# SNUCP/MKTFHE

Measured on AMD Instinct MI355X. Metric: NAND gate-bootstraps/sec, higher is better.
Workload: dtype f64

## Files before the change

mktfhe_amd/csrc/context.cpp:

```cpp
#include <hip/hip_runtime.h>

#include <algorithm>
#include <cstdio>
#include <cstdlib>
#include <cstring>
#include <string.h>
#include <cmath>
#include <memory>
#include <string>
#include <vector>

#include "device_api.h"
#include "device_mem.h"
#include "fft_device.h"
#include "host_internal.h"
#include "rng_chacha.h"
#include "../../include/mktfhe_ring_share.h"

using mktd::cplx;
using mkt::DevBuf;

namespace {
thread_local std::string g_create_error;

struct TimedSpan { int cls; hipEvent_t a, b; };

int env_int(const char *name, int dflt) { const char *v = getenv(name); return v ? atoi(v) : dflt; }
// ... 19 lines not shown
struct DevGuard {
    int prev = -1; bool ok = true;
    explicit DevGuard(int dev) { if (hipGetDevice(&prev) != hipSuccess) prev = -1; if (prev != dev) ok = hipSetDevice(dev) == hipSuccess; }
    ~DevGuard() { if (prev >= 0) (void)hipSetDevice(prev); }
};
Tune tune_from_env() { Tune t; for (const Switch &w : SWITCHES) t.*w.member = w.env ? env_int(w.env, w.dflt) : w.dflt; return t; }
}

thread_local const char *mktd::last_rot_kernel = "";
thread_local int mktd::last_rot_static_l = 0, mktd::last_rot_static_logB = 0;

const mktd::LaunchTuning &mktd::launch_tuning() {
    static const LaunchTuning t = [] {
        LaunchTuning q{};
        q.fft_grid = env_int("MKT_FFT_GRID", 0); q.fft_nb = env_int("MKT_FFT_NB", 1); q.fft_igrid = env_int("MKT_FFT_IGRID", 0);
        q.ks_g = env_int("MKT_KS_G", 32); q.ks_blocks = env_int("MKT_KS_BLOCKS", 0); q.ks_waves = env_int("MKT_KS_WAVES", 0); q.ks_pair = env_int("MKT_KS_PAIR", -1); q.ntt_grid = env_int("MKT_NTT_GRID", 0);
        return q;
    }();
    return t;
}

enum KeyTable { T_TW, T_MONOMIAL, T_BRK, T_KSK, T_PUB, T_CRS, T_RLK_D, T_RLK_F, T_SLOT_PARTY, T_SLOT_ROW, T_FX_TAB, T_FX_BRK, T_FX_STAT, T_NTT, T_COUNT };
struct ResidentTable {
    void **slot = nullptr; size_t elems = 0, esize = 0;
    bool per_party = false, present = false, cloned = false;
    size_t bytes(int nparty) const { return (per_party ? (size_t)nparty : 1) * elems * esize; }
};
struct KeySet {
    int device = 0;
    mkt::Twiddles tw;
    cplx *d_tw = nullptr;
    cplx *d_monomial = nullptr;
    cplx *d_brk = nullptr;
    uint32_t *d_ksk = nullptr; mkt::KskLayout ksk;
    cplx *d_rlk_d = nullptr, *d_rlk_f = nullptr, *d_pub = nullptr, *d_crs = nullptr;
    mkt::LoadedKeys loaded;
    int rtot = 1;
    int *d_slot_party = nullptr, *d_slot_row = nullptr;
    uint64_t *d_ntt = nullptr;
    cplx *d_fx_tab = nullptr;
    cplx *d_fx_brk = nullptr;
    unsigned long long *d_fx_stat = nullptr;
    double fx_kmax = 0.0;
    DevBuf d_pack; int pack_l = 0, pack_logB = 0; size_t pack_party_bytes = 0;
    std::vector<uint8_t> pack_loaded;
    ResidentTable tab[T_COUNT];
    DevBuf own[T_COUNT];
    size_t stride(KeyTable t) const { return tab[t].elems; }
    template <class T> T *party(KeyTable t, int party) const { return static_cast<T *>(*tab[t].slot) + (size_t)party * tab[t].elems; }
// ... 20 lines not shown
    int device = 0;
    int logM = 0, logN = 0, M = 0;
    int dev_order = MKT_DEVORDER;
    hipStream_t stream = nullptr;
    hipStream_t own_stream = nullptr;
    hipEvent_t moved = nullptr;
    std::string err;
    std::shared_ptr<KeySet> ks;
    bool exact = false;
    int split = 1;
    Workspace ws;
    bool timing = false;
    std::vector<TimedSpan> spans;
    Tune tune{};
    const char *last_rot_kernel = "";
    int rot_static_l = 0, rot_static_logB = 0;
    double pm_amax = 0.0;
    double pm_bound = -1.0;
    double fx_last_resid = 0.0;

    const cplx *fx_om() const { return ks->d_fx_tab; }
    const cplx *fx_tw() const { return ks->d_fx_tab + M; }
    const cplx *fx_nat() const { return ks->d_fx_tab + 2 * (size_t)M; }
    mktd::TwPtrs twp() const { return mktd::TwPtrs{ks->d_tw, ks->d_tw + M, ks->d_tw + 2 * (size_t)M, ks->d_tw + 3 * (size_t)M}; }
    bool keys_shared() const { return ks.use_count() > 1; }
};

namespace {

int fail(mkt_ctx *c, int code, const std::string &msg) { if (c) c->err = msg; else g_create_error = msg; return code; }
// ... 248 lines not shown
    mktd::RotArgs a = rot_args(c, lwe, stride, pre);
    a.init_mode = 0; a.out_mode = 0; a.acc_io = acc; a.ngates = B;
    if (route == Route::F64_KANY) HIPCHK(c, mktd::launch_blindrotate_kany(c->logM, p.W, p.k, a, scratch, B, c->stream));
    else if (route == Route::F64_KR) HIPCHK(c, mktd::launch_blindrotate_kr(c->logM, p.W, p.k, a, B, c->stream));
    else HIPCHK(c, mktd::launch_blindrotate_k1(c->logM, p.W, a, B, c->stream));
    return MKT_OK;
}

int do_keyswitch(mkt_ctx *c, const void *acc, uint32_t *out, size_t B, const uint32_t *src = nullptr, const uint32_t *coef = nullptr, size_t nacc = 0) {
    const mkt_params &p = c->p;
    mktd::KsArgs a{};
    a.src = src; a.coef = coef; a.nacc = nacc;
    a.acc = acc; a.out = out; a.ksk = c->ks->d_ksk; a.ksk_party_stride = c->ks->stride(T_KSK); a.n1p = c->ks->ksk.n1p;
    a.N = p.N; a.n = p.n; a.f = p.f; a.logD = p.logD; a.drows = c->sh.ksk_drows; a.kacc = c->sh.kacc;
    a.mk = mkt::is_mk(p.scheme) ? 1 : 0; a.balanced = mkt::is_block(p.scheme) ? 1 : 0; a.lmss = p.scheme == MKT_LMSS ? 1 : 0;
    size_t dw = 0, pw = 0;
    mktd::ks_scratch_words(a, B, &dw, &pw);
    HIPCHK(c, c->ws.ksd.reserve((dw + pw) * 4));
    if (dw) { a.digits = c->ws.ksd.as<uint32_t>(); a.partial = a.digits + dw; }
    Timer tm(c, 2);
    HIPCHK(c, mktd::launch_keyswitch(p.W, a, B, c->stream));
    return MKT_OK;
}

int rotate_chunk(mkt_ctx *c, const uint32_t *lin, size_t B) {
    const mkt_params &p = c->p;
    if (!mkt::is_kms(p.scheme)) {
        HIPCHK(c, mktd::launch_testvector(p.W, lin, c->sh.lwe_len, c->logN, c->sh.kacc, c->ws.acc.p, B, c->stream));
        return do_blindrotate(c, lin, c->sh.lwe_len, 0, nullptr, c->ws.acc.p, B);
    }
// ... 211 lines not shown
    auto row = [&](KeyTable t, auto &member, size_t elems, bool per_party, bool present, bool cloned) { ks.tab[t] = ResidentTable{(void **)&member, elems, sizeof(*member), per_party, present, cloned}; };
    row(T_TW,         ks.d_tw,         4 * M,                                                         false,     true,    true);
    row(T_MONOMIAL,   ks.d_monomial,   2 * N * M,                                                     false,     true,    true);
    row(T_BRK,        ks.d_brk,        (size_t)p.n * c->sh.brk_polys * tp,                            true,      true,    true);
    row(T_KSK,        ks.d_ksk,        ks.ksk.resident_words(),                                        true,      true,    true);
    row(T_PUB,        ks.d_pub,        (size_t)p.l_uni * tp,                                          true,      mk,      true);
    row(T_CRS,        ks.d_crs,        (size_t)p.l_uni * tp,                                          false,     mk,      true);
    row(T_RLK_D,      ks.d_rlk_d,      (size_t)p.l_uni * tp,                                          true,      kms,     true);
    row(T_RLK_F,      ks.d_rlk_f,      (size_t)p.l_uni * 2 * tp,                                      true,      kms,     true);
    row(T_SLOT_PARTY, ks.d_slot_party, (size_t)ks.rtot,                                               false,     true,    false);
    row(T_SLOT_ROW,   ks.d_slot_row,   (size_t)ks.rtot,                                               false,     true,    false);
    row(T_FX_TAB,     ks.d_fx_tab,     3 * M,                                                         false,     fx,      false);
    row(T_FX_BRK,     ks.d_fx_brk,     fx_per,                                                        true,      fx,      true);
    row(T_FX_STAT,    ks.d_fx_stat,    1,                                                             false,     fx,      true);
    row(T_NTT,        ks.d_ntt,        (N + 4) * 2,                                                   false,     c->exact, false);
}

constexpr int NO_PARTY = -1; enum class Gate { EXACT, F64_OR_EXACT_KMS };
int key_write_guard(mkt_ctx *c, bool ptrs_ok, int party, Gate gate, bool (*scheme_ok)(int) = nullptr) {
    if (!c || !ptrs_ok || (party != NO_PARTY && (party < 0 || party >= c->sh.nparty)) || (scheme_ok && !scheme_ok(c->p.scheme))) return fail(c, MKT_ERR_ARG, "bad argument");
    if (gate == Gate::EXACT) MKT_EXACT_GATE(c); else MKT_F64_OR_EXACT_KMS(c);
    return keys_writable(c);
}
hipError_t install_brk(mkt_ctx *c, int party, const void *src) {
    KeySet &ks = *c->ks;
    hipError_t e = to_resident(c, src, mkt::brk_polys_total(c->p, c->sh), ks.party<cplx>(T_BRK, party), false, ks.d_fx_brk ? ks.party<cplx>(T_FX_BRK, party) : nullptr);
    if (e == hipSuccess) e = hipStreamSynchronize(c->stream);
    if (e == hipSuccess && ks.d_fx_brk) e = fx_after_key_load(c);
    if (e == hipSuccess) ks.loaded.mark(mkt::K_BRK, party);
    return e;
}
hipError_t ksk_zero(mkt_ctx *c, int party) { return hipMemsetAsync(c->ks->party<uint32_t>(T_KSK, party), 0, c->ks->stride(T_KSK) * sizeof(uint32_t), c->stream); }
hipError_t ksk_repitch(mkt_ctx *c, uint32_t *dst, int dpitch, const uint32_t *src, int spitch, hipMemcpyKind kind) { return hipMemcpy2DAsync(dst, (size_t)dpitch * 4, src, (size_t)spitch * 4, (size_t)c->ks->ksk.n1 * 4, c->ks->ksk.rows, kind, c->stream); }
hipError_t ksk_to_resident(mkt_ctx *c, int party, const uint32_t *rows, hipMemcpyKind kind) { return ksk_repitch(c, c->ks->party<uint32_t>(T_KSK, party), c->ks->ksk.n1p, rows, c->ks->ksk.n1, kind); }
hipError_t ksk_to_rows(mkt_ctx *c, const uint32_t *padded, uint32_t *rows, hipMemcpyKind kind) { return ksk_repitch(c, rows, c->ks->ksk.n1, padded, c->ks->ksk.n1p, kind); }

}

extern "C" {

int mkt_abi_version(void) { return MKT_ABI_VERSION; }

const char *mkt_last_error(const mkt_ctx *ctx) { return ctx ? ctx->err.c_str() : g_create_error.c_str(); }

int mkt_ctx_create(const mkt_params *params, int arith_mode, int device, mkt_ctx **out) {
    if (!params || !out) return fail(nullptr, MKT_ERR_ARG, "null argument");
    *out = nullptr;
    std::string why;
    if (mkt::validate_params(*params, why)) return fail(nullptr, MKT_ERR_ARG, why);
    if (arith_mode != MKT_ARITH_F64REF && arith_mode != MKT_ARITH_EXACT) return fail(nullptr, MKT_ERR_ARG, "unknown arithmetic mode");
// ... 25 lines not shown
    DevGuard dg(device);
    auto bail = [&](int code) { std::string m = c->err; mkt_ctx_destroy(c); g_create_error = m; return code; };
    if (!dg.ok) { c->err = "hipSetDevice failed"; return bail(MKT_ERR_HIP); }
    const mkt_params &p = c->p;
    const int np = c->sh.nparty, M = c->M;
    c->ks->loaded.reset(np);
    mkt::make_twiddles(p.N, c->ks->tw);
    std::vector<int> sp, sr;
    if (mkt::is_kms(p.scheme)) {
        for (int i = 0; i < p.k; i++) { int rows = i == 0 ? 1 : p.l_lev; for (int r = 0; r < rows; r++) { sp.push_back(i); sr.push_back(r); } }
    } else { sp.push_back(0); sr.push_back(0); }
    c->ks->rtot = (int)sp.size();
    describe_key_set(c);
    if (c->ks->stride(T_BRK) * sizeof(cplx) > 0x7fffffffull) { c->err = "per-party bootstrapping key exceeds the 2 GiB window of the rotation kernels' buffer descriptors"; return bail(MKT_ERR_UNSUPPORTED); }
#define CK(call) do { hipError_t _e = (call); if (_e != hipSuccess) { c->err = std::string(#call) + ": " + hipGetErrorString(_e); return bail(_e == hipErrorOutOfMemory ? MKT_ERR_NOMEM : MKT_ERR_HIP); } } while (0)
    for (int t = 0; t < T_COUNT; t++) if (c->ks->tab[t].present) { CK(c->ks->own[t].alloc(c->ks->tab[t].bytes(np))); *c->ks->tab[t].slot = c->ks->own[t].p; }
    CK(hipMemcpy(c->ks->d_slot_party, sp.data(), sp.size() * sizeof(int), hipMemcpyHostToDevice));
    CK(hipMemcpy(c->ks->d_slot_row, sr.data(), sr.size() * sizeof(int), hipMemcpyHostToDevice));
    if (c->ks->d_fx_tab) {
        CK(hipMemset(c->ks->d_fx_stat, 0, 8));
        const size_t tb = (size_t)M * sizeof(cplx);
        CK(hipMemcpy(c->ks->d_fx_tab, c->ks->tw.fx_om.data(), tb, hipMemcpyHostToDevice));
        CK(hipMemcpy(c->ks->d_fx_tab + M, c->ks->tw.fx_tw.data(), tb, hipMemcpyHostToDevice));
        CK(hipMemcpy(c->ks->d_fx_tab + 2 * (size_t)M, c->ks->tw.fx_nat.data(), tb, hipMemcpyHostToDevice));
    }
#undef CK
    int r = upload_twiddles(c);
    if (!r && c->exact) r = upload_ntt_tables(c);
    if (!r) r = build_monomial(c);
    if (r) return bail(r);
    *out = c;
// ... 44 lines not shown
    if (!src || !dst) return MKT_ERR_ARG;
    if (std::memcmp(&src->p, &dst->p, sizeof(mkt_params)) != 0 || src->exact != dst->exact) return fail(dst, MKT_ERR_ARG, "key replication between contexts of different parameters");
    if (int w = keys_writable(dst)) return w;
    { DevGuard g(src->device); HIPCHK(dst, hipStreamSynchronize(src->stream)); }
    const int sd = src->device, dd = dst->device;
    KeySet &a = *src->ks, &b = *dst->ks;
    b.tw = a.tw;
    for (int t = 0; t < T_COUNT; t++)
        if (a.tab[t].cloned && a.tab[t].present && b.tab[t].present)
            HIPCHK(dst, (hipError_t)mkt_internal_copy_across(*b.tab[t].slot, dd, *a.tab[t].slot, sd, a.tab[t].bytes(src->sh.nparty), no_peer));
    if (a.d_fx_brk && b.d_fx_brk) b.fx_kmax = a.fx_kmax;
    b.loaded = a.loaded;
    dst->tune = src->tune;
    { DevGuard g(sd); HIPCHK(dst, hipDeviceSynchronize()); }
    { DevGuard g(dd); HIPCHK(dst, hipDeviceSynchronize()); }
    return MKT_OK;
}
#ifndef MKT_BUILD_ID
#define MKT_BUILD_ID "unknown"
#endif
const char *mkt_build_id(void) { return MKT_BUILD_ID; }
int mkt_internal_device_of(const mkt_ctx *c) { return c ? c->device : -1; }
size_t mkt_internal_lwe_len(const mkt_ctx *c) { return c ? (size_t)c->sh.lwe_len : 0; }
size_t mkt_internal_acc_bytes(const mkt_ctx *c) { return c ? (size_t)(1 + c->sh.kacc) * poly_bytes(c) : 0; }

int mkt_set_stream(mkt_ctx *c, void *hip_stream) {
    if (!c) return MKT_ERR_ARG;
    const hipStream_t next = (hipStream_t)hip_stream;
    if (next == c->stream) return MKT_OK;
    DevGuard dg(c->device);
    if (!c->moved) HIPCHK(c, hipEventCreateWithFlags(&c->moved, hipEventDisableTiming));
    HIPCHK(c, hipEventRecord(c->moved, c->stream));
// ... 15 lines not shown
            return fail(c, MKT_ERR_ARG, "mkt_set_option: " + k + " = " + std::to_string(value) + " is not one of " + list);
        }
        if (w.resets_workspace && c->tune.*w.member != value) c->ws.gates = 0;
        c->tune.*w.member = value;
        return MKT_OK;
    }
    return fail(c, MKT_ERR_ARG, "mkt_set_option: unknown option '" + k + "'");
}

const char *mkt_last_kernel_name(const mkt_ctx *c) { return c ? c->last_rot_kernel : ""; }

int mkt_get_metric(mkt_ctx *c, const char *name, double *out) {
    if (!c || !name || !out) return fail(c, MKT_ERR_ARG, "null argument");
    const std::string k(name);
    if (k == "fx_available") *out = fx_usable(c) ? 1.0 : 0.0;
    else if (k == "fx_bound") *out = c->ks->d_fx_brk ? fx_bound(c, c->ks->fx_kmax) : -1.0;
    else if (k == "fx_kmax") *out = c->ks->fx_kmax;
    else if (k == "fx_last_resid") *out = c->fx_last_resid;
    else if (k == "polymul_amax") *out = c->pm_amax;
    else if (k == "fx_polymul_bound") *out = c->pm_bound;
    else if (k == "rot_static_l") *out = c->rot_static_l;
    else if (k == "rot_static_logB") *out = c->rot_static_logB;
    else if (k == "mem_guard_check") {
        DevGuard dg(c->device);
        *out = (double)mkt::memguard::sweep(c->device);
        mkt::memguard::Finding f;
        if (mkt::memguard::last_finding(f)) c->err = mkt::memguard::text(f);
    }
    else if (k == "mem_guard_buffers") *out = (double)mkt::memguard::swept();
    else if (k == "mem_guard_released") *out = (double)mkt::memguard::released();
// ... 51 lines not shown
}

int mkt_load_brk(mkt_ctx *c, int party, const void *data, int fmt) {
    if (int r = key_write_guard(c, data != nullptr, party, Gate::EXACT)) return r;
    DevGuard dg(c->device);
    int r = upload_polys(c, data, mkt::brk_polys_total(c->p, c->sh), c->ks->party<cplx>(T_BRK, party), fmt, false, party);
    if (!r && fmt != MKT_FMT_INT_COEFF) c->ks->loaded.mark(mkt::K_BRK, party);
    return r;
}

int mkt_load_ksk(mkt_ctx *c, int party, const uint32_t *data) {
    if (int r = key_write_guard(c, data != nullptr, party, Gate::EXACT)) return r;
    DevGuard dg(c->device);
    HIPCHK(c, ksk_zero(c, party));
    HIPCHK(c, ksk_to_resident(c, party, data, hipMemcpyHostToDevice));
    HIPCHK(c, hipStreamSynchronize(c->stream));
    c->ks->loaded.mark(mkt::K_KSK, party);
    return MKT_OK;
}

int mkt_load_rlk(mkt_ctx *c, int party, const void *d, const void *f, int fmt) {
    if (int r = key_write_guard(c, d && f, party, Gate::F64_OR_EXACT_KMS, mkt::is_kms)) return r;
    DevGuard dg(c->device);
    const size_t l = (size_t)c->p.l_uni;
    int r = upload_polys(c, d, l, c->ks->party<cplx>(T_RLK_D, party), fmt);
    if (!r) r = upload_polys(c, f, 2 * l, c->ks->party<cplx>(T_RLK_F, party), fmt);
    if (!r) c->ks->loaded.mark(mkt::K_RLK, party);
    return r;
}

// ... 22 lines not shown
    DevGuard dg(c->device);
    const size_t brk_bytes = mkt::brk_polys_total(p, c->sh) * poly_bytes(c);
    DevBuf out, crs_int;
    DeviceSecret lwe{c}, z{c};
    mktd::KeygenArgs a{};
    hipError_t e = keygen_setup(c, K, crs, lwe, z, {{&out, brk_bytes}}, crs_int, a);
    if (e != hipSuccess) return hipfail(c, e, "device keygen setup");
    a.out = out.p; a.zoff = 0;
    if (!ring_keys_cover(c, K)) e = hipErrorInvalidValue;
    if (e == hipSuccess) e = mktd::launch_keygen_brk(a, unienc ? 1 : 0, c->stream);
    if (e == hipSuccess && brk_out) e = hipMemcpyAsync(brk_out, out.p, brk_bytes, hipMemcpyDeviceToHost, c->stream);
    if (e == hipSuccess) e = install_brk(c, party, out.p);
    if (e == hipSuccess) e = ksk_zero(c, party);
    a.zoff = mkt::is_kms(p.scheme) ? 1 : 0;
    if (e == hipSuccess) e = mktd::launch_keygen_ksk(a, c->ks->party<uint32_t>(T_KSK, party), c->ks->ksk.n1p, c->sh.ksk_kr, c->sh.ksk_drows, mkt::is_block(p.scheme) ? 1 : 0, c->stream);
    e = wipe_secrets(wipe_secrets(e, z, a), lwe, a);
    if (e != hipSuccess) return hipfail(c, e, "device keygen");
    c->ks->loaded.mark(mkt::K_KSK, party);
    if (ksk_out) return mkt_get_ksk(c, party, ksk_out);
    return MKT_OK;
}

int mkt_keygen_device(mkt_ctx *c, int party, const mkt_client_party *K, const void *crs) {
    return keygen_device_impl(c, party, K, crs, nullptr, nullptr);
}

int mkt_keygen_device_export(mkt_ctx *c, int party, const mkt_client_party *K, const void *crs, void *brk_out, uint32_t *ksk_out) {
    if (!brk_out || !ksk_out) return fail(c, MKT_ERR_ARG, "null output");
    return keygen_device_impl(c, party, K, crs, brk_out, ksk_out);
}
// ... 86 lines not shown
        a.log_units = c->logN + (p.W == 64 ? 1 : 0) - 4; a.body = sb.dev; a.out = dst; a.npolys = brk_polys_total;
        e = mktd::launch_seeded_brk_expand(a, c->stream);
        if (e == hipSuccess && load) e = install_brk(c, party, dst);
        if (e != hipSuccess) return hipfail(c, e, "seeded bootstrapping key expansion");
    }
    if (ksk_seeded) {
        if ((r = sk.in(ksk_seeded, rows * 4, mem, true))) return r;
        uint32_t *dst = c->ks->party<uint32_t>(T_KSK, party);
        if (!load) { HIPCHK(c, padded.alloc(c->ks->ksk.resident_words() * 4)); dst = padded.as<uint32_t>(); }
        mktd::SeededKskArgs a{};
        mkt::seed_to_key(mask_seed, a.mkey);
        a.party = party; a.n = p.n; a.n1p = c->ks->ksk.n1p; a.rows_per_cj = (uint32_t)(c->sh.ksk_drows * p.f);
        a.absent_below = mkt::is_block(p.scheme) ? p.n : 0; a.body = sk.as<const uint32_t>(); a.out = dst; a.rows = rows;
        e = mktd::launch_seeded_ksk_expand(a, c->stream);
        if (e == hipSuccess && !load) e = ksk_to_rows(c, dst, ksk_out, mem == MKT_MEM_HOST ? hipMemcpyDeviceToHost : hipMemcpyDeviceToDevice);
        if (e != hipSuccess) return hipfail(c, e, "seeded key-switching key expansion");
    }
    HIPCHK(c, hipStreamSynchronize(c->stream));
    if (!load) return brk_out ? so.out(brk_out) : MKT_OK;
    if (ksk_seeded) c->ks->loaded.mark(mkt::K_KSK, party);
    return MKT_OK;
}

int mkt_seeded_keys_expand(mkt_ctx *c, int party, const uint8_t *mask_seed, const void *brk_seeded, const uint32_t *ksk_seeded, void *brk_out, uint32_t *ksk_out, int mem) {
    return seeded_keys_impl(c, party, mask_seed, brk_seeded, ksk_seeded, false, brk_out, ksk_out, mem);
}

int mkt_load_seeded_keys(mkt_ctx *c, int party, const uint8_t *mask_seed, const void *brk_seeded, const uint32_t *ksk_seeded) {
    if (int r = key_write_guard(c, brk_seeded || ksk_seeded, NO_PARTY, Gate::EXACT)) return r;
    return seeded_keys_impl(c, party, mask_seed, brk_seeded, ksk_seeded, true, nullptr, nullptr, MKT_MEM_HOST);
// ... 791 lines not shown
```

mktfhe_amd/csrc/device_api.h:

```cpp
#pragma once
#include <hip/hip_runtime.h>
#include <stddef.h>
#include <stdint.h>

#include "rot_plan.h"

namespace mktd {

struct cplx;

struct TwPtrs { const cplx *psi, *psiinv, *roots, *rootsinv; };

struct LaunchTuning { int fft_grid, fft_nb, fft_igrid, ks_g, ks_blocks, ks_waves, ks_pair, ntt_grid; };
const LaunchTuning &launch_tuning();
extern thread_local const char *last_rot_kernel;
extern thread_local int last_rot_static_l, last_rot_static_logB;
inline void note_rot_kernel(const char *name, int static_l = 0, int static_logB = 0) {
    last_rot_kernel = name; last_rot_static_l = static_l; last_rot_static_logB = static_logB;
}

struct RotArgs {
    TwPtrs tw;
    const cplx *brk;
    size_t brk_party_stride;
    const cplx *monomial;
    const uint32_t *lwe;
    int lwe_stride;
    int pre_switched;
// ... 43 lines not shown
    const uint32_t *lwe;
    int lwe_stride, pre_switched;
    int n, logN, k, l, logB;
    const cplx *brk;
    size_t brk_party_stride;
    const cplx *pub_b;
    const cplx *crs;
    const cplx *monomial;
    void *acc;
    cplx *scratch;
    void *vscratch;
    int stagger;
    int dev_order;
};

struct KsArgs {
    const void *acc;
    uint32_t *out;
    const uint32_t *ksk;
    size_t ksk_party_stride;
    int n1p;
    int N, n, f, logD, drows;
    int kacc;
    int mk;
    int balanced;
    int lmss;
    uint32_t *digits;
    uint32_t *partial;
    const uint32_t *src;
    const uint32_t *coef;
    size_t nacc;
};
void ks_scratch_words(const KsArgs &a, size_t B, size_t *digit_words, size_t *partial_words);

struct KeygenArgs {
    uint32_t key[8];
    int party;
    int N, n, W;
    int kr, l, logB;
    int zoff;
    int f, logD;
    double sigma_ring, sigma_lwe;
    const uint32_t *lwekey;
    const int8_t *zring;
    const void *crs;
    void *out;
};
hipError_t launch_keygen_brk(const KeygenArgs &a, int unienc, hipStream_t s);
// ... 228 lines not shown
```

mktfhe_amd/csrc/host_internal.h:

```cpp
#pragma once
#include <cstddef>
#include <cstdint>
#include <cstring>
#include <string>
#include <vector>

#include "../../include/mktfhe.h"
#include "../../include/mktfhe_pack.h"

namespace mkt {

struct Twiddles {
    std::vector<double> psi, psiinv, roots, rootsinv;
    std::vector<double> fx_om, fx_tw, fx_nat;
};
void make_twiddles(int N, Twiddles &tw);

inline bool is_mk(int s) { return s == MKT_CCS || s == MKT_KMS || s == MKT_KMS_BLOCK; }
inline bool is_kms(int s) { return s == MKT_KMS || s == MKT_KMS_BLOCK; }
inline bool is_block(int s) { return s == MKT_LMSS || s == MKT_KMS_BLOCK; }

struct Shape {
    int nparty;
    int kr;
// ... 24 lines not shown
inline bool lut_nout_ok(int nout, int N) { return (nout == 1 || nout == 2 || nout == 4 || nout == 8) && nout <= N; }
inline bool lut_nu_ok(int nu, int N) { return nu >= 0 && nu <= 3 && (1 << nu) <= N; }
inline bool lut_ncoef_ok(size_t ncoef, int N) { return ncoef >= 1 && ncoef <= (size_t)N; }
inline bool host_below(const uint32_t *v, size_t n, size_t bound) {
    for (size_t j = 0; j < n; j++) if (v[j] >= bound) return false;
    return true;
}
inline size_t brk_seeded_polys(const mkt_params &p, const Shape &s) { return (size_t)p.n * (p.scheme == MKT_CCS ? 2 * (size_t)p.l_uni : (size_t)(s.kr + 1) * p.l_gsw); }
inline size_t ksk_rows(const mkt_params &p, const Shape &s) { return (size_t)s.ksk_kr * p.N * s.ksk_drows * p.f; }
inline size_t brk_polys_total(const mkt_params &p, const Shape &s) { return (size_t)p.n * s.brk_polys; }
struct KskLayout {
    size_t rows = 0; int n1 = 0, n1p = 0;
    size_t resident_words() const { return rows * (size_t)n1p; }
};
inline KskLayout ksk_layout(const mkt_params &p, const Shape &s) { return KskLayout{ksk_rows(p, s), p.n + 1, (p.n + 1 + 3) / 4 * 4}; }

enum KeyPiece { K_BRK, K_KSK, K_RLK, K_PUB, K_CRS };
struct LoadedKeys {
    std::vector<uint8_t> of;
    static constexpr unsigned bit(KeyPiece k) { return 1u << k; }
    void reset(int nparty) { of.assign((size_t)nparty, 0); }
    void mark(KeyPiece k, int party) { for (size_t i = 0; i < of.size(); i++) if (party < 0 || (size_t)party == i) of[i] |= (uint8_t)bit(k); }
    bool has_all(unsigned pieces, int party) const { return (of[(size_t)party] & pieces) == pieces; }
    bool has(KeyPiece k, int party) const { return has_all(bit(k), party < 0 ? 0 : party); }
    bool any_transformed() const {
        for (uint8_t m : of) if (m & (bit(K_BRK) | bit(K_RLK) | bit(K_PUB) | bit(K_CRS))) return true;
        return false;
    }
};
inline bool pack_gadget_ok(int l, int logB) { return logB >= 1 && logB <= 16 && l >= 1 && l * logB <= 32; }
// ... 40 lines not shown
```

mktfhe_amd/csrc/kernels.hip:

```cpp
#include "kernel_common.h"

#include <type_traits>

#pragma clang fp contract(off)

#ifdef MKT_TU
#define MKT_IN_TU(n) (MKT_TU == (n))
#else
#define MKT_IN_TU(n) 1
#endif

namespace mktd {

#if MKT_IN_TU(0)
constexpr int FFT_PF = 2;
typedef double __attribute__((ext_vector_type(2))) mkt_d2;
template <typename T> __device__ __forceinline__ T stream_load(const T *p) { return __builtin_nontemporal_load(p); }
__device__ __forceinline__ cplx stream_load_c(const cplx *p) {
    mkt_d2 v = __builtin_nontemporal_load(reinterpret_cast<const mkt_d2 *>(p));
    return cplx{v.x, v.y};
}
__device__ __forceinline__ void stream_store_c(cplx *p, cplx z) {
    mkt_d2 v = {z.re, z.im};
    __builtin_nontemporal_store(v, reinterpret_cast<mkt_d2 *>(p));
// ... 1567 lines not shown
        if (W == 64) return launch_ccs_one<LM, uint64_t, 0, 0>(a, B, s);
        if constexpr (LM == 9 || LM == 10) {
            if (a.l == 3 && a.logB == 8) return launch_ccs_one<LM, uint32_t, 3, 8>(a, B, s);
            if (a.l == 4 && a.logB == 8) return launch_ccs_one<LM, uint32_t, 4, 8>(a, B, s);
            if (a.l == 5 && a.logB == 6) return launch_ccs_one<LM, uint32_t, 5, 6>(a, B, s);
        }
        return launch_ccs_one<LM, uint32_t, 0, 0>(a, B, s);
    });
    return hipGetLastError();
}

#endif

#if MKT_IN_TU(0)
namespace {
struct KsPlan { int G, waves, ngroups, parties, gblocks, slabs, jslab; bool pair; };
KsPlan ks_plan(const KsArgs &a, size_t B, bool have_scratch) {
    KsPlan q{};
    q.G = 32;
    int target_blocks = 1024;
    if (a.balanced) target_blocks = a.mk ? 4096 : 8192;
    const LaunchTuning &lt = launch_tuning();
    if (lt.ks_g == 8 || lt.ks_g == 16) q.G = lt.ks_g;
    if (lt.ks_blocks > 0) target_blocks = lt.ks_blocks;
    q.pair = lt.ks_pair != 0 && a.logD == 2 && a.f % 2 == 0 && q.G == 32 && have_scratch;
    if (q.pair && lt.ks_blocks <= 0) target_blocks = 1024;
    q.ngroups = (int)((B + q.G - 1) / q.G);
    q.parties = a.mk ? a.kacc : 1;
    auto nslabs = [&] {
        int sl = (target_blocks + q.ngroups * q.parties - 1) / (q.ngroups * q.parties);
        if (sl < 1) sl = 1;
        if (sl > a.N / 8) sl = a.N / 8;
        return sl < 1 ? 1 : sl;
    };
    q.slabs = nslabs();
    q.jslab = (a.N + q.slabs - 1) / q.slabs;
    q.slabs = (a.N + q.jslab - 1) / q.jslab;
    q.waves = lt.ks_waves > 0 ? lt.ks_waves : 4;
    if (q.waves != 2 && q.waves != 4) q.waves = 1;
    if (q.G != 32) q.waves = 1;
    if (a.balanced && lt.ks_waves <= 0 && !q.pair) q.waves = 1;
    q.gblocks = (q.ngroups + q.waves - 1) / q.waves;
    return q;
}
}

void ks_scratch_words(const KsArgs &a, size_t B, size_t *digit_words, size_t *partial_words) {
    const KsPlan q = ks_plan(a, B, true);
    *digit_words = q.pair ? (size_t)a.kacc * q.ngroups * (size_t)a.N * 32 : 0;
    *partial_words = q.pair ? (size_t)q.slabs * q.parties * B * (size_t)a.n1p : 0;
}

template <bool AT>
static hipError_t launch_keyswitch_as(int W, const KsArgs &a, size_t B, hipStream_t s) {
    const KsPlan q = ks_plan(a, B, a.digits && a.partial);
    const int ngroups = q.ngroups;
    const dim3 grid((unsigned)(q.gblocks * q.slabs), (unsigned)q.parties, (unsigned)((a.n1p + KS_CHUNK_WORDS - 1) / KS_CHUNK_WORDS));
    const size_t ks_lds = q.pair ? (size_t)KS_STAGES * 16 * KS_LANES * sizeof(uint4) : (size_t)KS_STAGES * (1 + a.drows * (a.balanced ? 2 : 1)) * KS_LANES * sizeof(uint4);
    if (ks_lds > 64 * 1024) return hipErrorInvalidValue;
    const dim3 words(blocks_for(B * (size_t)ks_lwe_len(a), 256));
    using C1 = std::integral_constant<int, 1>; using C2 = std::integral_constant<int, 2>; using C4 = std::integral_constant<int, 4>;
    auto with_word = [&](auto f) { if (W == 64) f(uint64_t{}); else f(uint32_t{}); };
    auto with_bal = [&](auto f) { if (a.balanced) f(std::true_type{}); else f(std::false_type{}); };
    auto with_waves = [&](auto f) { if (q.waves == 4) f(C4{}); else if (q.waves == 2) f(C2{}); else f(C1{}); };
    if (q.pair) {
        const dim3 dgrid((unsigned)((a.N + 7) / 8), (unsigned)ngroups, (unsigned)a.kacc);
        with_word([&](auto w) { with_bal([&](auto bal) {
            hipLaunchKernelGGL((ks_digits_kernel<decltype(w), decltype(bal)::value, AT>), dgrid, dim3(256), 0, s, a, (int)B, ngroups);
        }); });
        with_bal([&](auto bal) { with_waves([&](auto wv) {
            hipLaunchKernelGGL((keyswitch_pair_kernel<32, decltype(wv)::value, decltype(bal)::value>), grid, dim3(KS_LANES * decltype(wv)::value), ks_lds, s, a, (int)B, ngroups);
        }); });
        with_word([&](auto w) { hipLaunchKernelGGL((ks_reduce_kernel<decltype(w), AT>), words, dim3(256), 0, s, a, B, q.slabs, q.parties); });
        return hipGetLastError();
    }
    with_word([&](auto w) {
        hipLaunchKernelGGL((ks_init_kernel<decltype(w), AT>), words, dim3(256), 0, s, a, B);
        with_bal([&](auto bal) {
            auto mg = [&](auto g, auto wv) {
// ... 184 lines not shown
```

Baseline: 60140.

## Compute key-switch sums with int8 MFMA over byte-plane packed key-switching keys

Adds an alternative key-switching path. The key-switching key is repacked at load or keygen time into signed int8 byte planes. The digit-times-key accumulation then runs as 32x32x32 int8 MFMA matrix multiplies, with a 6-slot register ring prefetching key planes and digit words, split into slabs sized to fill the compute units. The existing digit extraction and reduce kernels are reused. This replaces the scalar/LDS multiply-accumulate in the keyswitch with matrix-core throughput, at the cost of extra device memory for the plane copy and a heuristic slab split.

```diff
diff --git a/mktfhe_amd/csrc/context.cpp b/mktfhe_amd/csrc/context.cpp
--- a/mktfhe_amd/csrc/context.cpp
+++ b/mktfhe_amd/csrc/context.cpp
@@ -11,6 +11,7 @@
 #include <vector>
 
 #include "device_api.h"
+#include "ks_mfma.h"
 #include "device_mem.h"
 #include "fft_device.h"
 #include "host_internal.h"
@@ -60,13 +61,13 @@
     static const LaunchTuning t = [] {
         LaunchTuning q{};
         q.fft_grid = env_int("MKT_FFT_GRID", 0); q.fft_nb = env_int("MKT_FFT_NB", 1); q.fft_igrid = env_int("MKT_FFT_IGRID", 0);
-        q.ks_g = env_int("MKT_KS_G", 32); q.ks_blocks = env_int("MKT_KS_BLOCKS", 0); q.ks_waves = env_int("MKT_KS_WAVES", 0); q.ks_pair = env_int("MKT_KS_PAIR", -1); q.ntt_grid = env_int("MKT_NTT_GRID", 0);
+        q.ks_g = env_int("MKT_KS_G", 32); q.ks_blocks = env_int("MKT_KS_BLOCKS", 0); q.ks_waves = env_int("MKT_KS_WAVES", 0); q.ks_pair = env_int("MKT_KS_PAIR", -1); q.ks_mfma = env_int("MKT_KS_MFMA", -1); q.ntt_grid = env_int("MKT_NTT_GRID", 0);
         return q;
     }();
     return t;
 }
 
-enum KeyTable { T_TW, T_MONOMIAL, T_BRK, T_KSK, T_PUB, T_CRS, T_RLK_D, T_RLK_F, T_SLOT_PARTY, T_SLOT_ROW, T_FX_TAB, T_FX_BRK, T_FX_STAT, T_NTT, T_COUNT };
+enum KeyTable { T_TW, T_MONOMIAL, T_BRK, T_KSK, T_PUB, T_CRS, T_RLK_D, T_RLK_F, T_SLOT_PARTY, T_SLOT_ROW, T_FX_TAB, T_FX_BRK, T_FX_STAT, T_NTT, T_KSK_PLANES, T_COUNT };
 struct ResidentTable {
     void **slot = nullptr; size_t elems = 0, esize = 0;
     bool per_party = false, present = false, cloned = false;
@@ -79,6 +80,7 @@
     cplx *d_monomial = nullptr;
     cplx *d_brk = nullptr;
     uint32_t *d_ksk = nullptr; mkt::KskLayout ksk;
+    int8_t *d_ksk_planes = nullptr;
     cplx *d_rlk_d = nullptr, *d_rlk_f = nullptr, *d_pub = nullptr, *d_crs = nullptr;
     mkt::LoadedKeys loaded;
     int rtot = 1;
@@ -129,6 +131,7 @@
     std::vector<TimedSpan> spans;
     Tune tune{};
     const char *last_rot_kernel = "";
+    int ks_mfma_last = 0;
     int rot_static_l = 0, rot_static_logB = 0;
     double pm_amax = 0.0;
     double pm_bound = -1.0;
@@ -407,6 +410,8 @@
     a.acc = acc; a.out = out; a.ksk = c->ks->d_ksk; a.ksk_party_stride = c->ks->stride(T_KSK); a.n1p = c->ks->ksk.n1p;
     a.N = p.N; a.n = p.n; a.f = p.f; a.logD = p.logD; a.drows = c->sh.ksk_drows; a.kacc = c->sh.kacc;
     a.mk = mkt::is_mk(p.scheme) ? 1 : 0; a.balanced = mkt::is_block(p.scheme) ? 1 : 0; a.lmss = p.scheme == MKT_LMSS ? 1 : 0;
+    a.planes = c->ks->d_ksk_planes; a.sum_mfma = mktd::launch_ks_mfma; a.planes_block_stride = mktd::ksm_block_bytes(p.N, p.f, a.n1p);
+    c->ks_mfma_last = mktd::ks_uses_mfma(a, B);
     size_t dw = 0, pw = 0;
     mktd::ks_scratch_words(a, B, &dw, &pw);
     HIPCHK(c, c->ws.ksd.reserve((dw + pw) * 4));
@@ -648,6 +653,9 @@
     row(T_FX_BRK,     ks.d_fx_brk,     fx_per,                                                        true,      fx,      true);
     row(T_FX_STAT,    ks.d_fx_stat,    1,                                                             false,     fx,      true);
     row(T_NTT,        ks.d_ntt,        (N + 4) * 2,                                                   false,     c->exact, false);
+    const bool planes = mktd::launch_tuning().ks_mfma != 0 && p.logD == 2 && !mkt::is_block(p.scheme) && c->sh.ksk_drows == 3 && (!mk || c->sh.ksk_kr == 1) &&
+                        mkt::ks_mfma_fits(p.N, mk ? 1 : c->sh.kacc, p.f);
+    row(T_KSK_PLANES, ks.d_ksk_planes, (size_t)c->sh.ksk_kr * mktd::ksm_block_bytes(p.N, p.f, ks.ksk.n1p),   true,      planes,   true);
 }
 
 constexpr int NO_PARTY = -1; enum class Gate { EXACT, F64_OR_EXACT_KMS };
@@ -668,6 +676,15 @@
 hipError_t ksk_repitch(mkt_ctx *c, uint32_t *dst, int dpitch, const uint32_t *src, int spitch, hipMemcpyKind kind) { return hipMemcpy2DAsync(dst, (size_t)dpitch * 4, src, (size_t)spitch * 4, (size_t)c->ks->ksk.n1 * 4, c->ks->ksk.rows, kind, c->stream); }
 hipError_t ksk_to_resident(mkt_ctx *c, int party, const uint32_t *rows, hipMemcpyKind kind) { return ksk_repitch(c, c->ks->party<uint32_t>(T_KSK, party), c->ks->ksk.n1p, rows, c->ks->ksk.n1, kind); }
 hipError_t ksk_to_rows(mkt_ctx *c, const uint32_t *padded, uint32_t *rows, hipMemcpyKind kind) { return ksk_repitch(c, rows, c->ks->ksk.n1, padded, c->ks->ksk.n1p, kind); }
+hipError_t ksk_to_planes(mkt_ctx *c, int party) {
+    KeySet &ks = *c->ks;
+    if (!ks.d_ksk_planes) return hipSuccess;
+    const size_t comp_words = (size_t)c->p.N * c->sh.ksk_drows * c->p.f * ks.ksk.n1p, block = mktd::ksm_block_bytes(c->p.N, c->p.f, ks.ksk.n1p);
+    for (int comp = 0; comp < c->sh.ksk_kr; comp++)
+        if (hipError_t e = mktd::launch_ks_mfma_pack(ks.party<uint32_t>(T_KSK, party) + comp * comp_words, ks.party<int8_t>(T_KSK_PLANES, party) + comp * block,
+                                                     c->p.N, c->p.f, c->sh.ksk_drows, ks.ksk.n1p, c->stream); e != hipSuccess) return e;
+    return hipSuccess;
+}
 
 }
 
@@ -723,7 +740,11 @@
     describe_key_set(c);
     if (c->ks->stride(T_BRK) * sizeof(cplx) > 0x7fffffffull) { c->err = "per-party bootstrapping key exceeds the 2 GiB window of the rotation kernels' buffer descriptors"; return bail(MKT_ERR_UNSUPPORTED); }
 #define CK(call) do { hipError_t _e = (call); if (_e != hipSuccess) { c->err = std::string(#call) + ": " + hipGetErrorString(_e); return bail(_e == hipErrorOutOfMemory ? MKT_ERR_NOMEM : MKT_ERR_HIP); } } while (0)
-    for (int t = 0; t < T_COUNT; t++) if (c->ks->tab[t].present) { CK(c->ks->own[t].alloc(c->ks->tab[t].bytes(np))); *c->ks->tab[t].slot = c->ks->own[t].p; }
+    for (int t = 0; t < T_COUNT; t++) if (c->ks->tab[t].present) {
+        if (t == T_KSK_PLANES && c->ks->own[t].alloc(c->ks->tab[t].bytes(np)) != hipSuccess) { (void)hipGetLastError(); c->ks->tab[t].present = false; continue; }
+        if (t != T_KSK_PLANES) CK(c->ks->own[t].alloc(c->ks->tab[t].bytes(np)));
+        *c->ks->tab[t].slot = c->ks->own[t].p;
+    }
     CK(hipMemcpy(c->ks->d_slot_party, sp.data(), sp.size() * sizeof(int), hipMemcpyHostToDevice));
     CK(hipMemcpy(c->ks->d_slot_row, sr.data(), sr.size() * sizeof(int), hipMemcpyHostToDevice));
     if (c->ks->d_fx_tab) {
@@ -798,8 +819,20 @@
     dst->tune = src->tune;
     { DevGuard g(sd); HIPCHK(dst, hipDeviceSynchronize()); }
     { DevGuard g(dd); HIPCHK(dst, hipDeviceSynchronize()); }
-    return MKT_OK;
-}
+    if (b.d_ksk_planes && !a.d_ksk_planes) {
+        DevGuard g(dd);
+        for (int party = 0; party < dst->sh.nparty; party++) if (b.loaded.has(mkt::K_KSK, party)) HIPCHK(dst, ksk_to_planes(dst, party));
+        HIPCHK(dst, hipStreamSynchronize(dst->stream));
+    }
+    return MKT_OK;
+}
+size_t mkt_internal_ks_mfma_block_bytes(int N, int f, int n1p) { return mktd::ksm_block_bytes(N, f, n1p); }
+void mkt_internal_ks_mfma_pack_host(const uint32_t *rows, int N, int f, int drows, int n1p, int8_t *planes) {
+    const size_t bytes = mktd::ksm_block_bytes(N, f, n1p);
+    for (size_t off = 0; off < bytes; off++) planes[off] = mktd::ksm_plane_byte(rows, N, f, drows, n1p, off);
+}
+int mkt_internal_ks_mfma_fits(long long N, long long kr, long long f) { return mkt::ks_mfma_fits(N, kr, f) ? 1 : 0; }
+int mkt_internal_ks_mfma_env(void) { return env_int("MKT_KS_MFMA", -1); }
 #ifndef MKT_BUILD_ID
 #define MKT_BUILD_ID "unknown"
 #endif
@@ -845,6 +878,9 @@
     if (!c || !name || !out) return fail(c, MKT_ERR_ARG, "null argument");
     const std::string k(name);
     if (k == "fx_available") *out = fx_usable(c) ? 1.0 : 0.0;
+    else if (k == "ks_mfma") *out = mktd::launch_tuning().ks_mfma;
+    else if (k == "ks_mfma_planes") *out = c->ks->d_ksk_planes ? 1.0 : 0.0;
+    else if (k == "ks_mfma_last") *out = c->ks_mfma_last;
     else if (k == "fx_bound") *out = c->ks->d_fx_brk ? fx_bound(c, c->ks->fx_kmax) : -1.0;
     else if (k == "fx_kmax") *out = c->ks->fx_kmax;
     else if (k == "fx_last_resid") *out = c->fx_last_resid;
@@ -926,6 +962,7 @@
     DevGuard dg(c->device);
     HIPCHK(c, ksk_zero(c, party));
     HIPCHK(c, ksk_to_resident(c, party, data, hipMemcpyHostToDevice));
+    HIPCHK(c, ksk_to_planes(c, party));
     HIPCHK(c, hipStreamSynchronize(c->stream));
     c->ks->loaded.mark(mkt::K_KSK, party);
     return MKT_OK;
@@ -978,6 +1015,7 @@
     if (e == hipSuccess) e = ksk_zero(c, party);
     a.zoff = mkt::is_kms(p.scheme) ? 1 : 0;
     if (e == hipSuccess) e = mktd::launch_keygen_ksk(a, c->ks->party<uint32_t>(T_KSK, party), c->ks->ksk.n1p, c->sh.ksk_kr, c->sh.ksk_drows, mkt::is_block(p.scheme) ? 1 : 0, c->stream);
+    if (e == hipSuccess) e = ksk_to_planes(c, party);
     e = wipe_secrets(wipe_secrets(e, z, a), lwe, a);
     if (e != hipSuccess) return hipfail(c, e, "device keygen");
     c->ks->loaded.mark(mkt::K_KSK, party);
@@ -1094,6 +1132,7 @@
         a.absent_below = mkt::is_block(p.scheme) ? p.n : 0; a.body = sk.as<const uint32_t>(); a.out = dst; a.rows = rows;
         e = mktd::launch_seeded_ksk_expand(a, c->stream);
         if (e == hipSuccess && !load) e = ksk_to_rows(c, dst, ksk_out, mem == MKT_MEM_HOST ? hipMemcpyDeviceToHost : hipMemcpyDeviceToDevice);
+        if (e == hipSuccess && load) e = ksk_to_planes(c, party);
         if (e != hipSuccess) return hipfail(c, e, "seeded key-switching key expansion");
     }
     HIPCHK(c, hipStreamSynchronize(c->stream));
diff --git a/mktfhe_amd/csrc/device_api.h b/mktfhe_amd/csrc/device_api.h
--- a/mktfhe_amd/csrc/device_api.h
+++ b/mktfhe_amd/csrc/device_api.h
@@ -11,7 +11,7 @@
 
 struct TwPtrs { const cplx *psi, *psiinv, *roots, *rootsinv; };
 
-struct LaunchTuning { int fft_grid, fft_nb, fft_igrid, ks_g, ks_blocks, ks_waves, ks_pair, ntt_grid; };
+struct LaunchTuning { int fft_grid, fft_nb, fft_igrid, ks_g, ks_blocks, ks_waves, ks_pair, ntt_grid, ks_mfma; };
 const LaunchTuning &launch_tuning();
 extern thread_local const char *last_rot_kernel;
 extern thread_local int last_rot_static_l, last_rot_static_logB;
@@ -85,6 +85,7 @@
     int dev_order;
 };
 
+struct KsmArgs;
 struct KsArgs {
     const void *acc;
     uint32_t *out;
@@ -101,8 +102,15 @@
     const uint32_t *src;
     const uint32_t *coef;
     size_t nacc;
+    const int8_t *planes;
+    size_t planes_block_stride;
+    hipError_t (*sum_mfma)(const struct KsmArgs &, hipStream_t);
 };
 void ks_scratch_words(const KsArgs &a, size_t B, size_t *digit_words, size_t *partial_words);
+int ks_uses_mfma(const KsArgs &a, size_t B);
+struct KsmArgs;
+hipError_t launch_ks_mfma_pack(const uint32_t *rows, int8_t *planes, int N, int f, int drows, int n1p, hipStream_t s);
+hipError_t launch_ks_mfma(const KsmArgs &a, hipStream_t s);
 
 struct KeygenArgs {
     uint32_t key[8];
diff --git a/mktfhe_amd/csrc/host_internal.h b/mktfhe_amd/csrc/host_internal.h
--- a/mktfhe_amd/csrc/host_internal.h
+++ b/mktfhe_amd/csrc/host_internal.h
@@ -62,6 +62,7 @@
     size_t resident_words() const { return rows * (size_t)n1p; }
 };
 inline KskLayout ksk_layout(const mkt_params &p, const Shape &s) { return KskLayout{ksk_rows(p, s), p.n + 1, (p.n + 1 + 3) / 4 * 4}; }
+inline bool ks_mfma_fits(long long N, long long kr, long long f) { return N > 0 && kr > 0 && f > 0 && N * kr * f * 255 < (1ll << 31); }
 
 enum KeyPiece { K_BRK, K_KSK, K_RLK, K_PUB, K_CRS };
 struct LoadedKeys {
diff --git a/mktfhe_amd/csrc/kernels.hip b/mktfhe_amd/csrc/kernels.hip
--- a/mktfhe_amd/csrc/kernels.hip
+++ b/mktfhe_amd/csrc/kernels.hip
@@ -1,4 +1,5 @@
 #include "kernel_common.h"
+#include "ks_mfma.h"
 
 #include <type_traits>
 
@@ -1605,7 +1606,9 @@
 
 #if MKT_IN_TU(0)
 namespace {
-struct KsPlan { int G, waves, ngroups, parties, gblocks, slabs, jslab; bool pair; };
+struct KsPlan { int G, waves, ngroups, parties, gblocks, slabs, jslab; bool pair, mfma; };
+constexpr int KS_MFMA_MIN_BATCH = 1;
+constexpr int KS_MFMA_CUS = 256;
 KsPlan ks_plan(const KsArgs &a, size_t B, bool have_scratch) {
     KsPlan q{};
     q.G = 32;
@@ -1616,8 +1619,26 @@
     if (lt.ks_blocks > 0) target_blocks = lt.ks_blocks;
     q.pair = lt.ks_pair != 0 && a.logD == 2 && a.f % 2 == 0 && q.G == 32 && have_scratch;
     if (q.pair && lt.ks_blocks <= 0) target_blocks = 1024;
+    q.parties = a.mk ? a.kacc : 1;
+    q.mfma = a.sum_mfma && lt.ks_mfma != 0 && a.planes && !a.balanced && a.logD == 2 && a.drows == 3 && have_scratch && (lt.ks_mfma > 0 || B >= (size_t)KS_MFMA_MIN_BATCH);
+    if (q.mfma) {
+        q.G = 32; q.waves = KSM_WAVES; q.pair = false;
+        q.ngroups = (int)((B + 31) / 32);
+        const int gtiles = (int)((B + KSM_WAVE_GATES * KSM_WAVES - 1) / (KSM_WAVE_GATES * KSM_WAVES));
+        const int per_slab = gtiles * q.parties * ksm_coltiles(a.n1p);
+        int most = ksm_steps(a.N, a.f) / KSM_RING;
+        if (most < 1) most = 1;
+        int first = 2 * KS_MFMA_CUS / per_slab;
+        first = first < 1 ? 1 : (first > most ? most : first);
+        q.slabs = first;
+        for (int sl = first; sl <= most && sl < first + 8; sl++) {
+            const long wg = (long)per_slab * sl, rounds = (wg + KS_MFMA_CUS - 1) / KS_MFMA_CUS;
+            if (wg * 10 >= rounds * KS_MFMA_CUS * 9) { q.slabs = sl; break; }
+        }
+        q.gblocks = gtiles; q.jslab = 0;
+        return q;
+    }
     q.ngroups = (int)((B + q.G - 1) / q.G);
-    q.parties = a.mk ? a.kacc : 1;
     auto nslabs = [&] {
         int sl = (target_blocks + q.ngroups * q.parties - 1) / (q.ngroups * q.parties);
         if (sl < 1) sl = 1;
@@ -1638,9 +1659,11 @@
 
 void ks_scratch_words(const KsArgs &a, size_t B, size_t *digit_words, size_t *partial_words) {
     const KsPlan q = ks_plan(a, B, true);
-    *digit_words = q.pair ? (size_t)a.kacc * q.ngroups * (size_t)a.N * 32 : 0;
-    *partial_words = q.pair ? (size_t)q.slabs * q.parties * B * (size_t)a.n1p : 0;
-}
+    const bool scratch = q.pair || q.mfma;
+    *digit_words = scratch ? (size_t)a.kacc * q.ngroups * (size_t)a.N * 32 : 0;
+    *partial_words = scratch ? (size_t)q.slabs * q.parties * B * (size_t)a.n1p : 0;
+}
+int ks_uses_mfma(const KsArgs &a, size_t B) { return B && ks_plan(a, B, true).mfma ? 1 : 0; }
 
 template <bool AT>
 static hipError_t launch_keyswitch_as(int W, const KsArgs &a, size_t B, hipStream_t s) {
@@ -1654,6 +1677,14 @@
     auto with_word = [&](auto f) { if (W == 64) f(uint64_t{}); else f(uint32_t{}); };
     auto with_bal = [&](auto f) { if (a.balanced) f(std::true_type{}); else f(std::false_type{}); };
     auto with_waves = [&](auto f) { if (q.waves == 4) f(C4{}); else if (q.waves == 2) f(C2{}); else f(C1{}); };
+    if (q.mfma) {
+        const dim3 dgrid((unsigned)((a.N + 7) / 8), (unsigned)ngroups, (unsigned)a.kacc);
+        with_word([&](auto w) { hipLaunchKernelGGL((ks_digits_kernel<decltype(w), false, AT>), dgrid, dim3(256), 0, s, a, (int)B, ngroups); });
+        const KsmArgs m{a.planes, a.planes_block_stride, a.digits, a.partial, (int)B, ngroups, a.N, a.f, a.n1p, a.kacc, a.mk, q.slabs};
+        if (hipError_t e = a.sum_mfma(m, s); e != hipSuccess) return e;
+        with_word([&](auto w) { hipLaunchKernelGGL((ks_reduce_kernel<decltype(w), AT>), words, dim3(256), 0, s, a, B, q.slabs, q.parties); });
+        return hipGetLastError();
+    }
     if (q.pair) {
         const dim3 dgrid((unsigned)((a.N + 7) / 8), (unsigned)ngroups, (unsigned)a.kacc);
         with_word([&](auto w) { with_bal([&](auto bal) {
diff --git a/mktfhe_amd/csrc/ks_mfma.h b/mktfhe_amd/csrc/ks_mfma.h
--- /dev/null
+++ b/mktfhe_amd/csrc/ks_mfma.h
@@ -0,0 +1,177 @@
+#pragma once
+#include <stddef.h>
+#include <stdint.h>
+#include <type_traits>
+
+#ifndef __HIPCC__
+#define KSM_HD inline
+#else
+#include <hip/hip_runtime.h>
+#define KSM_HD __host__ __device__ inline
+#endif
+
+namespace mktd {
+
+constexpr int KSM_STEP_DIGITS = 8;
+constexpr int KSM_TILE_WORDS = 32;
+constexpr int KSM_BLOCK_BYTES = 4096;
+constexpr int KSM_WAVE_GATES = 128;
+constexpr int KSM_WAVES = 4;
+
+KSM_HD int ksm_steps(int N, int f) { return (N * f + KSM_STEP_DIGITS - 1) / KSM_STEP_DIGITS; }
+KSM_HD int ksm_coltiles(int n1p) { return (n1p + KSM_TILE_WORDS - 1) / KSM_TILE_WORDS; }
+KSM_HD size_t ksm_block_bytes(int N, int f, int n1p) { return (size_t)ksm_steps(N, f) * ksm_coltiles(n1p) * KSM_BLOCK_BYTES; }
+
+KSM_HD int ksm_byte(uint32_t w, int b) {
+    for (int i = 0; i < b; i++) w = (w - (uint32_t)(int32_t)(int8_t)(w & 0xFF)) >> 8;
+    return (int8_t)(w & 0xFF);
+}
+
+KSM_HD int8_t ksm_plane_byte(const uint32_t *rows, int N, int f, int drows, int n1p, size_t off) {
+    const int coltiles = ksm_coltiles(n1p);
+    const size_t blk = off / KSM_BLOCK_BYTES;
+    const int o = (int)(off % KSM_BLOCK_BYTES);
+    const int step = (int)(blk / coltiles), tile = (int)(blk % coltiles);
+    const int plane = o >> 10, lane = (o >> 4) & 63, e = o & 15;
+    const int q = tile * KSM_TILE_WORDS + (lane & 31), d = e & 3;
+    const long s = (long)step * KSM_STEP_DIGITS + 4 * (lane >> 5) + (e >> 2);
+    if (d == 0 || d > drows || s >= (long)N * f || q >= n1p) return 0;
+    const int j = (int)(s / f), t = (int)(s % f);
+    return (int8_t)ksm_byte(rows[(((size_t)j * drows + (d - 1)) * f + t) * n1p + q], plane);
+}
+
+struct KsmArgs {
+    const int8_t *planes;
+    size_t block_stride;
+    const uint32_t *digits;
+    uint32_t *partial;
+    int B, ngroups, N, f, n1p, kacc, mk, slabs;
+};
+
+#ifdef __HIPCC__
+typedef int ksm_v4 __attribute__((ext_vector_type(4)));
+typedef int ksm_v16 __attribute__((ext_vector_type(16)));
+
+template <int F>
+__device__ __forceinline__ uint32_t ksm_digit_word(const uint32_t *dg, int step, int h, int N, int f) {
+    if constexpr (F == 8) return dg[(size_t)step * 32];
+    else {
+        uint32_t b8 = 0;
+#pragma unroll
+        for (int i = 0; i < 4; i++) {
+            const int s = step * KSM_STEP_DIGITS + 4 * h + i;
+            uint32_t d = 0;
+            if (s < N * f) { const int j = s / f, t = s - j * f; d = (dg[(size_t)j * 32] >> (2 * (f - 1 - t))) & 3u; }
+            b8 = (b8 << 2) | d;
+        }
+        return b8;
+    }
+}
+__device__ __forceinline__ ksm_v4 ksm_a_operand(uint32_t w, int sh) {
+    ksm_v4 v;
+#pragma unroll
+    for (int i = 0; i < 4; i++) v[i] = (int)(1u << (((w >> (sh + 6 - 2 * i)) & 3u) << 3));
+    return v;
+}
+
+constexpr int KSM_RING = 6;
+template <int F>
+__device__ __forceinline__ void ksm_tile_loop(const KsmArgs &a, ksm_v16 (&sum)[4][4], int grp0, int tile, int c_begin, int c_end, int s0, int s1) {
+    constexpr int R = KSM_RING;
+    const int lane = threadIdx.x & 63, r = lane & 31, h = lane >> 5;
+    const int f = F ? F : a.f, sh = F == 8 ? 8 * (1 - h) : 0;
+    const size_t step_bytes = (size_t)ksm_coltiles(a.n1p) * KSM_BLOCK_BYTES;
+    if (s0 >= s1) return;
+    for (int c = c_begin; c < c_end; c++) {
+        const int8_t *pl = a.planes + (size_t)c * a.block_stride + (size_t)tile * KSM_BLOCK_BYTES + (size_t)lane * 16;
+        const uint32_t *dg[4];
+#pragma unroll
+        for (int m = 0; m < 4; m++) {
+            const int grp = grp0 + m < a.ngroups ? grp0 + m : a.ngroups - 1;
+            dg[m] = a.digits + ((size_t)c * a.ngroups + grp) * a.N * 32 + r;
+        }
+        const int last = s1 - 1;
+        auto clamp = [=](int s) { return s < last ? s : last; };
+        ksm_v4 bv[R][4], av[2][4];
+        uint32_t w[R][4];
+        uint32_t w0[4];
+#pragma unroll
+        for (int m = 0; m < 4; m++) w0[m] = ksm_digit_word<F>(dg[m], s0, h, a.N, f);
+#pragma unroll
+        for (int k = 0; k < R - 1; k++) {
+            asm volatile("" ::: "memory");
+            __builtin_amdgcn_sched_barrier(0);
+#pragma unroll
+            for (int p = 0; p < 4; p++) bv[k][p] = *reinterpret_cast<const ksm_v4 *>(pl + (size_t)clamp(s0 + k) * step_bytes + p * 1024);
+#pragma unroll
+            for (int m = 0; m < 4; m++) w[k + 1][m] = ksm_digit_word<F>(dg[m], clamp(s0 + k + 1), h, a.N, f);
+        }
+        asm volatile("" ::: "memory");
+        __builtin_amdgcn_sched_barrier(0);
+#pragma unroll
+        for (int m = 0; m < 4; m++) av[0][m] = ksm_a_operand(w0[m], sh);
+        auto one_step = [&](auto slot, int step) {
+            constexpr int I = decltype(slot)::value, PREV = (I + R - 1) % R, NEXT = (I + 1) % R;
+            const int nb = clamp(step + R - 1), nw = clamp(step + R);
+#pragma unroll
+            for (int p = 0; p < 4; p++) bv[PREV][p] = *reinterpret_cast<const ksm_v4 *>(pl + (size_t)nb * step_bytes + p * 1024);
+#pragma unroll
+            for (int m = 0; m < 4; m++) w[I][m] = ksm_digit_word<F>(dg[m], nw, h, a.N, f);
+            asm volatile("" ::: "memory");
+            __builtin_amdgcn_sched_barrier(0);
+            const uint32_t live = step + 1 <= last ? ~0u : 0u;
+#pragma unroll
+            for (int m = 0; m < 4; m++) av[(I + 1) & 1][m] = ksm_a_operand(w[NEXT][m] & live, sh);
+#pragma unroll
+            for (int m = 0; m < 4; m++)
+#pragma unroll
+                for (int p = 0; p < 4; p++) sum[m][p] = __builtin_amdgcn_mfma_i32_32x32x32_i8(av[I & 1][m], bv[I][p], sum[m][p], 0, 0, 0);
+#pragma unroll
+            for (int m = 0; m < 4; m++) asm volatile("" : "+v"(av[(I + 1) & 1][m]));
+        };
+        for (int step = s0; step < s1; step += R) {
+            one_step(std::integral_constant<int, 0>{}, step);
+            one_step(std::integral_constant<int, 1>{}, step + 1);
+            one_step(std::integral_constant<int, 2>{}, step + 2);
+            one_step(std::integral_constant<int, 3>{}, step + 3);
+            one_step(std::integral_constant<int, 4>{}, step + 4);
+            one_step(std::integral_constant<int, 5>{}, step + 5);
+        }
+        static_assert(R == 6, "the loop above names every ring slot");
+    }
+}
+
+template <int F>
+__device__ __forceinline__ void ksm_workgroup(const KsmArgs &a) {
+    const int lane = threadIdx.x & 63, r = lane & 31, h = lane >> 5;
+    const int wv = __builtin_amdgcn_readfirstlane((int)(threadIdx.x >> 6));
+    const int gtiles = (a.B + KSM_WAVE_GATES * KSM_WAVES - 1) / (KSM_WAVE_GATES * KSM_WAVES);
+    const int gt = (int)(blockIdx.x % (unsigned)gtiles), slab = (int)(blockIdx.x / (unsigned)gtiles);
+    const int g0 = (gt * KSM_WAVES + wv) * KSM_WAVE_GATES;
+    if (g0 >= a.B) return;
+    const int tile = blockIdx.z;
+    const int c_begin = a.mk ? (int)blockIdx.y : 0, c_end = a.mk ? c_begin + 1 : a.kacc, blk = a.mk ? c_begin : 0;
+    const int nsteps = ksm_steps(a.N, F ? F : a.f), per = (nsteps + a.slabs - 1) / a.slabs;
+    const int s0 = slab * per, s1 = s0 + per < nsteps ? s0 + per : nsteps;
+    ksm_v16 sum[4][4];
+#pragma unroll
+    for (int m = 0; m < 4; m++)
+#pragma unroll
+        for (int p = 0; p < 4; p++)
+#pragma unroll
+            for (int i = 0; i < 16; i++) sum[m][p][i] = 0;
+    ksm_tile_loop<F>(a, sum, g0 / 32, tile, c_begin, c_end, s0, s1);
+    const int q = tile * KSM_TILE_WORDS + r;
+    if (q >= a.n1p) return;
+    uint32_t *dst = a.partial + ((size_t)slab * gridDim.y + blk) * a.B * a.n1p + q;
+#pragma unroll
+    for (int m = 0; m < 4; m++)
+#pragma unroll
+        for (int i = 0; i < 16; i++) {
+            const int g = g0 + 32 * m + (i & 3) + 8 * (i >> 2) + 4 * h;
+            if (g < a.B) dst[(size_t)g * a.n1p] = (uint32_t)sum[m][0][i] + ((uint32_t)sum[m][1][i] << 8) + ((uint32_t)sum[m][2][i] << 16) + ((uint32_t)sum[m][3][i] << 24);
+        }
+}
+#endif
+
+}
diff --git a/mktfhe_amd/csrc/ks_mfma.hip b/mktfhe_amd/csrc/ks_mfma.hip
--- /dev/null
+++ b/mktfhe_amd/csrc/ks_mfma.hip
@@ -0,0 +1,33 @@
+#include "ks_mfma.h"
+#include "device_api.h"
+
+namespace mktd {
+
+__global__ __launch_bounds__(256) void ks_mfma_pack_kernel(const uint32_t *rows, int8_t *planes, int N, int f, int drows, int n1p, size_t bytes) {
+    const size_t off = ((size_t)blockIdx.x * blockDim.x + threadIdx.x) * 16;
+    if (off >= bytes) return;
+    uint32_t w[4] = {0, 0, 0, 0};
+#pragma unroll
+    for (int e = 0; e < 16; e++) w[e >> 2] |= (uint32_t)(uint8_t)ksm_plane_byte(rows, N, f, drows, n1p, off + e) << (8 * (e & 3));
+    *reinterpret_cast<uint4 *>(planes + off) = make_uint4(w[0], w[1], w[2], w[3]);
+}
+
+template <int F>
+__global__ __launch_bounds__(64 * KSM_WAVES, 1) void ks_mfma_kernel(const KsmArgs a) { ksm_workgroup<F>(a); }
+
+hipError_t launch_ks_mfma_pack(const uint32_t *rows, int8_t *planes, int N, int f, int drows, int n1p, hipStream_t s) {
+    const size_t bytes = ksm_block_bytes(N, f, n1p);
+    hipLaunchKernelGGL(ks_mfma_pack_kernel, dim3((unsigned)((bytes / 16 + 255) / 256)), dim3(256), 0, s, rows, planes, N, f, drows, n1p, bytes);
+    return hipGetLastError();
+}
+
+hipError_t launch_ks_mfma(const KsmArgs &a, hipStream_t s) {
+    if (a.B < 1 || a.slabs < 1) return hipErrorInvalidValue;
+    const int gtiles = (a.B + KSM_WAVE_GATES * KSM_WAVES - 1) / (KSM_WAVE_GATES * KSM_WAVES);
+    const dim3 grid((unsigned)(gtiles * a.slabs), (unsigned)(a.mk ? a.kacc : 1), (unsigned)ksm_coltiles(a.n1p));
+    if (a.f == 8) hipLaunchKernelGGL(ks_mfma_kernel<8>, grid, dim3(64 * KSM_WAVES), 0, s, a);
+    else hipLaunchKernelGGL(ks_mfma_kernel<0>, grid, dim3(64 * KSM_WAVES), 0, s, a);
+    return hipGetLastError();
+}
+
+}
```

Result: faster. 61120, median of 6 (+1.6%).
